# lmb-freiburg/flownet2

Hardware: AMD Instinct MI355X
Metric: image-pairs/sec FlowNetC forward at 448x320 (higher is better)
Workload: dtype f32

## Files before the change

flownet2_amd/csrc/conv_mfma.hip:

```cpp
#include "mfma_tile.hpp"

namespace fn2 {
namespace cv {

using namespace mfma;

struct Args {
  const float* in; const float* wp; const float* bias; float* out;
  int N, Cin, Hin, Win, in_ctot, in_c0;
  int Cout, Hout, Wout, out_ctot, out_c0;
  int pad;
  int nchunks;
  int ksteps;
  int tx, ty;
  int ng;
  unsigned total;
  unsigned nbig;
  float slope; int relu;
};

template <int KS_, int S_, int MW_, int NP_, int WM_, int WNX_, int WNY_, int CQ_, int P16_ = 0, int PIN_ = 0>
struct Cfg : Window<((P16_ ? 1 : 4) * WNY_ - 1) * S_ + KS_,
                    ((P16_ ? 16 : 4) * NP_ * WNX_ - 1) * S_ + KS_ + 4,
                    CQ_, WM_ * WNX_ * WNY_> {
  static constexpr int KS = KS_, S = S_, MW = MW_, NP = NP_, WM = WM_, WNX = WNX_, WNY = WNY_, CQ = CQ_, P16 = P16_;
  static constexpr int PIN = PIN_;
  static constexpr int NW = WM * WNX * WNY, THREADS = 64 * NW;
  static constexpr int PADL = 4;
  static constexpr int TW = (P16 ? 16 : 4) * NP * WNX, TH = (P16 ? 1 : 4) * WNY;
  static_assert(!P16 || (KS == 1 && S == 1), "row tiles are for 1x1 kernels");
  static_assert(Cfg::WR == (TH - 1) * S + KS && Cfg::WC == (TW - 1) * S + KS + PADL, "window of the tile");
  static constexpr int KSC = CQ * KS * KS;
  static constexpr int NBUFA = ring_depth(KSC);
  static_assert(KSC % NBUFA == 0, "ring phase must repeat per chunk");
  static_assert(2 * Cfg::BUF * 4 <= 160 * 1024, "LDS");
};

template <class K>
__device__ __forceinline__ void conv_body(const Args& a, int g, int bx, int by, int n) {
  static_assert(K::THREADS == 256, "launch bounds");
  extern __shared__ __attribute__((aligned(16))) float smem[];
  constexpr int KS = K::KS, S = K::S, MW = K::MW, NP = K::NP;
  const int tid = threadIdx.x, lane = tid & 63;
  const int wave = __builtin_amdgcn_readfirstlane(tid >> 6);
  const int wm = wave % K::WM, wnx = (wave / K::WM) % K::WNX, wny = wave / (K::WM * K::WNX);
  const int x0 = bx * K::TW, y0 = by * K::TH;

  const size_t plane = (size_t)a.Hin * a.Win;
  const __amdgpu_buffer_rsrc_t rs = nchw_rsrc(a.in, n, a.in_ctot, a.in_c0, a.Cin, plane);
  unsigned voff[K::RPW];
  window_plan<K>(voff, wave, lane, S * y0 - a.pad, S * x0 - K::PADL, a.Hin, a.Win, plane);
  const unsigned lds_base = (unsigned)(uintptr_t)(lds_ptr_t)smem;
  const unsigned chunk_bytes = 4u * 4u * K::CQ * (unsigned)plane;
  auto stage = [&](int chunk, int buf) { stage_chunk<K>(rs, voff, lds_base + 4u * (unsigned)(buf * K::BUF), wave, (unsigned)chunk * chunk_bytes); };

  const int kq = lane >> 4, p16 = lane & 15, py = K::P16 ? 0 : p16 >> 2, px = K::P16 ? p16 : p16 & 3;
  constexpr int PW = K::P16 ? 16 : 4, PH = K::P16 ? 1 : 4;
  const int bbase = kq * K::CS + (S * (PH * wny + py)) * K::RS + S * (PW * NP * wnx + px) + K::PADL - a.pad;
  using WV = typename WVec<MW>::T;
  const int cg0 = (g * K::WM + wm) * MW;
  const float* wl = weight_lane(a.wp, cg0, a.ksteps, lane);

  f32x4 acc[MW][NP];
#pragma unroll
  for (int j = 0; j < MW; ++j)
#pragma unroll
    for (int p = 0; p < NP; ++p) acc[j][p] = f32x4{0.f, 0.f, 0.f, 0.f};

  WV wreg[K::NBUFA];
  stage(0, 0);
#pragma unroll
  for (int i = 0; i < K::NBUFA - 1; ++i) wreg[i] = weight_load<MW>(wl, i);

  for (int c = 0; c < a.nchunks; ++c) {
    const int buf = c & 1;
    wait_vmcnt<K::NBUFA - 1>();
    __builtin_amdgcn_s_barrier();
    if (c + 1 < a.nchunks) stage(c + 1, buf ^ 1);
    const float* win = smem + buf * K::BUF + bbase;
    const int ks0 = c * K::KSC;
    if constexpr (K::PIN) {
      float b[2][NP];
      auto tap_off = [](int ks) { const int cq = ks / (KS * KS), ky = (ks / KS) % KS, kx = ks % KS; return cq * 4 * K::CS + ky * K::RS + kx; };
#pragma unroll
      for (int p = 0; p < NP; ++p) b[0][p] = win[tap_off(0) + PW * S * p];
      __builtin_amdgcn_sched_barrier(0);
#pragma unroll
      for (int ks = 0; ks < K::KSC; ++ks) {
        wreg[(ks + K::NBUFA - 1) % K::NBUFA] = weight_load<MW>(wl, ks0 + ks + K::NBUFA - 1);
        const WV w = wreg[ks % K::NBUFA];
#pragma unroll
        for (int p = 0; p < NP; ++p) {
#pragma unroll
          for (int j = 0; j < MW; ++j) acc[j][p] = __builtin_amdgcn_mfma_f32_16x16x4f32(b[ks & 1][p], wget<MW>(w, j), acc[j][p], 0, 0, 0);
          if (ks + 1 < K::KSC) b[(ks + 1) & 1][p] = win[tap_off(ks + 1 < K::KSC ? ks + 1 : ks) + PW * S * p];
          __builtin_amdgcn_sched_barrier(0);
        }
      }
    } else {
#pragma unroll
    for (int ks = 0; ks < K::KSC; ++ks) {
      wreg[(ks + K::NBUFA - 1) % K::NBUFA] = weight_load<MW>(wl, ks0 + ks + K::NBUFA - 1);
      const int cq = ks / (KS * KS), ky = (ks / KS) % KS, kx = ks % KS;
      float b[NP];
#pragma unroll
      for (int p = 0; p < NP; ++p) b[p] = win[cq * 4 * K::CS + ky * K::RS + kx + PW * S * p];
      const WV w = wreg[ks % K::NBUFA];
#pragma unroll
      for (int j = 0; j < MW; ++j)
#pragma unroll
        for (int p = 0; p < NP; ++p) acc[j][p] = __builtin_amdgcn_mfma_f32_16x16x4f32(b[p], wget<MW>(w, j), acc[j][p], 0, 0, 0);
    }
    }
  }

  const int y = K::P16 ? y0 + wny : y0 + 4 * wny + (lane >> 4);
  if (y < a.Hout) {
#pragma unroll
    for (int j = 0; j < MW; ++j) {
      const int co = 16 * (cg0 + j) + (lane & 15);
      const float bv = a.bias ? a.bias[co] : 0.f;
      float* orow = a.out + (((size_t)n * a.out_ctot + a.out_c0 + co) * a.Hout + y) * a.Wout;
#pragma unroll
      for (int p = 0; p < NP; ++p) {
        const int x = K::P16 ? x0 + 16 * (NP * wnx + p) + 4 * (lane >> 4) : x0 + 4 * (NP * wnx + p);
        store_row4(orow, x, a.Wout, acc[j][p], bv, a.relu, a.slope);
      }
    }
  }
}

__device__ __forceinline__ void decode_tile(const Args& a, unsigned t, int& g, int& bx, int& by, int& n) {
  g = t % a.ng; t /= a.ng;
  bx = t % a.tx; t /= a.tx;
  by = t % a.ty;
  n = t / a.ty;
}

template <class K>
__global__ void __launch_bounds__(256, 2)
conv_mfma(Args a) {
  unsigned t;
  if (!xcd_task(blockIdx.x, a.total, t)) return;
  int g, bx, by, n;
  decode_tile(a, t, g, bx, by, n);
  conv_body<K>(a, g, bx, by, n);
}

template <class K>
__global__ void __launch_bounds__(256, 2)
conv_mfma_tail(Args a) {
  using KH = Cfg<K::KS, K::S, K::MW / 2, K::NP, K::WM, K::WNX, K::WNY, K::CQ, K::P16>;
  int g, bx, by, n;
  if (blockIdx.x < a.nbig) {
    const unsigned t = (blockIdx.x % 8) * (a.nbig / 8) + blockIdx.x / 8;
    decode_tile(a, t, g, bx, by, n);
    conv_body<K>(a, g, bx, by, n);
  } else {
    unsigned u;
    if (!xcd_task(blockIdx.x - a.nbig, 2 * (a.total - a.nbig), u)) return;
    decode_tile(a, a.nbig + u / 2, g, bx, by, n);
    conv_body<KH>(a, 2 * g + (int)(u & 1), bx, by, n);
  }
}

__global__ void pack_weights(const float* __restrict__ w, float* __restrict__ wp, int Cout, int Cin, int KS, int ksteps, int kalloc) {
  const long long total = (long long)((Cout + 63) / 64) * kalloc * 256;
  for (long long i = blockIdx.x * (long long)blockDim.x + threadIdx.x; i < total; i += (long long)gridDim.x * blockDim.x) {
    const int j = (int)(i & 3), lane = (int)((i >> 2) & 63);
    long long r = i >> 8;
    const int ks = (int)(r % kalloc), grp = (int)(r / kalloc);
    const int co = 64 * grp + 16 * j + (lane & 15), kq = lane >> 4;
    const int cq = ks / (KS * KS), tap = ks % (KS * KS);
    const int ci = 4 * cq + kq;
    float v = 0.f;
    if (ks < ksteps && ci < Cin && co < Cout) v = w[((size_t)co * Cin + ci) * KS * KS + tap];
    wp[i] = v;
  }
}

template <int KS> struct PackTile {
  static constexpr int T = KS * KS;
  static constexpr int QT = KS == 1 ? 8 : KS == 3 ? 3 : KS == 4 ? 2 : 1;
  static constexpr int CIL = 4 * QT, ROW = CIL * T + 1;
  static constexpr int LDS_FLOATS = 64 * ROW;
};

template <int KS, int ORDER>
__global__ void __launch_bounds__(256) pack_weights_view(const float* __restrict__ w, float* __restrict__ wp, int ksteps, int kalloc,
                                                         int src_co, int src_ci, long long s_co, long long s_ci, int flip) {
  using P = PackTile<KS>;
  constexpr int T = P::T, QT = P::QT, CIL = P::CIL, ROW = P::ROW;
  __shared__ float tile[P::LDS_FLOATS];
  const int grp = blockIdx.x, cq0 = blockIdx.y * QT;
  const int co0 = 64 * grp, ci0 = 4 * cq0;
  const int nquads = ksteps / T;
  constexpr int TOTAL = 64 * CIL * T;
  if constexpr (ORDER == 0) {
    const float* src = w + (size_t)co0 * s_co + (size_t)ci0 * T;
#pragma unroll
    for (int i = threadIdx.x; i < TOTAL; i += 256) {
      const int col = i / (CIL * T), e = i - col * (CIL * T), c = e / T;
      tile[col * ROW + e] = (co0 + col < src_co && ci0 + c < src_ci) ? src[(size_t)col * s_co + e] : 0.f;
    }
  } else if constexpr (ORDER == 1) {
    const float* src = w + (size_t)ci0 * s_ci + (size_t)co0 * T;
#pragma unroll
    for (int i = threadIdx.x; i < TOTAL; i += 256) {
      const int c = i / (64 * T), e = i - c * (64 * T), col = e / T, t = e - col * T;
      tile[col * ROW + c * T + t] = (co0 + col < src_co && ci0 + c < src_ci) ? src[(size_t)c * s_ci + e] : 0.f;
    }
  } else {
#pragma unroll
    for (int i = threadIdx.x; i < TOTAL; i += 256) {
      const int col = i / (CIL * T), e = i - col * (CIL * T), c = e / T, t = e - c * T;
      tile[col * ROW + e] = (co0 + col < src_co && ci0 + c < src_ci) ? w[(size_t)(co0 + col) * s_co + (size_t)(ci0 + c) * s_ci + t] : 0.f;
    }
  }
  __syncthreads();
  const int nq = min(QT, nquads - cq0);
  float* dst = wp + ((size_t)grp * kalloc + (size_t)cq0 * T) * 256;
  const int j = threadIdx.x & 3, lane = threadIdx.x >> 2;
  const float* trow = tile + (16 * j + (lane & 15)) * ROW + (lane >> 4) * T;
#pragma unroll
  for (int ks = 0; ks < QT * T; ++ks) {
    const int cq = ks / T, tap = ks - cq * T;
    if (cq < nq) dst[ks * 256 + threadIdx.x] = trow[4 * cq * T + (flip ? T - 1 - tap : tap)];
  }
  if (cq0 + QT >= nquads)
    for (int i = threadIdx.x; i < (kalloc - ksteps) * 256; i += 256) wp[((size_t)grp * kalloc + ksteps) * 256 + i] = 0.f;
}

template <int KS>
static void launch_pack_view(const float* w, float* wp, int Cout, int ksteps, int kalloc, int src_co, int src_ci, long long s_co, long long s_ci, int flip,
                             hipStream_t st) {
  using P = PackTile<KS>;
  const dim3 grid((unsigned)((Cout + 63) / 64), (unsigned)cdiv(ksteps / P::T, P::QT));
  if (s_ci == (long long)P::T) hipLaunchKernelGGL((pack_weights_view<KS, 0>), grid, dim3(256), 0, st, w, wp, ksteps, kalloc, src_co, src_ci, s_co, s_ci, flip);
  else if (s_co == (long long)P::T) hipLaunchKernelGGL((pack_weights_view<KS, 1>), grid, dim3(256), 0, st, w, wp, ksteps, kalloc, src_co, src_ci, s_co, s_ci, flip);
  else hipLaunchKernelGGL((pack_weights_view<KS, 2>), grid, dim3(256), 0, st, w, wp, ksteps, kalloc, src_co, src_ci, s_co, s_ci, flip);
}

constexpr int kSpare = 8;
constexpr int kChunkQuads = 2;

inline int chunk_quads(int KS) { return KS == 1 ? 8 : kChunkQuads; }
inline int ksteps_for(int Cin, int KS) { return cdiv(cdiv(Cin, 4), chunk_quads(KS)) * chunk_quads(KS) * KS * KS; }

template <class K>
static void set_geometry(Args& a) {
  if constexpr (K::P16) {
    a.Win *= a.Hin; a.Hin = 1; a.Wout *= a.Hout; a.Hout = 1;
  }
  a.tx = cdiv(a.Wout, K::TW); a.ty = cdiv(a.Hout, K::TH);
  a.ng = a.Cout / (16 * K::MW * K::WM);
  a.nchunks = cdiv(cdiv(a.Cin, 4), K::CQ);
}

inline long long tiles_of(const Args& a) { return (long long)a.N * a.tx * a.ty * a.ng; }

template <class K>
static int launch(const Args& base, hipStream_t st) {
  Args a = base;
  set_geometry<K>(a);
  if (tiles_of(a) > 0x3fffff00ll) return fail(FN2_ERR_UNSUPPORTED, "conv_mfma: grid too large");
  a.total = (unsigned)tiles_of(a); a.nbig = a.total;
  const unsigned grid = 8 * ((a.total + 7) / 8);
  constexpr size_t lds = sizeof(float) * 2 * K::BUF;
  set_dynamic_lds_once<&conv_mfma<K>>((int)lds);
  hipLaunchKernelGGL((conv_mfma<K>), dim3(grid), dim3(K::THREADS), lds, st, a);
  return check_launch("conv_mfma_forward");
}

inline unsigned whole_rounds(long long tiles) { return (unsigned)(tiles / 256 * 256); }

template <class K>
static int launch_tail(const Args& base, hipStream_t st) {
  if constexpr (K::MW < 2) {
    return fail(FN2_ERR_UNSUPPORTED, "conv_mfma: variant has no split tail");
  } else {
    Args a = base;
    set_geometry<K>(a);
    if (tiles_of(a) > 0x1fffff00ll) return fail(FN2_ERR_UNSUPPORTED, "conv_mfma: grid too large");
    a.total = (unsigned)tiles_of(a); a.nbig = whole_rounds(a.total);
    const unsigned nsm = 2 * (a.total - a.nbig);
    const unsigned grid = a.nbig + 8 * ((nsm + 7) / 8);
    constexpr size_t lds = sizeof(float) * 2 * K::BUF;
    set_dynamic_lds_once<&conv_mfma_tail<K>>((int)lds);
    hipLaunchKernelGGL((conv_mfma_tail<K>), dim3(grid), dim3(K::THREADS), lds, st, a);
    return check_launch("conv_mfma_forward");
  }
}

struct Variant {
  int ks, s, mw, np, wm, wnx, wny, p16;
  int (*fn)(const Args&, hipStream_t);
  int (*fn_tail)(const Args&, hipStream_t);
};

#define FN2_CV_LIST(X) \
   \
  X(1, 1, 2, 7, 2, 2, 1, 8, 1) X(1, 1, 2, 7, 2, 1, 2, 8, 1) X(1, 1, 4, 7, 1, 2, 2, 8, 0) X(1, 1, 4, 7, 1, 1, 4, 8, 0) X(1, 1, 2, 6, 2, 2, 1, 8, 1) \
  X(1, 1, 2, 4, 2, 2, 1, 8, 1) X(1, 1, 2, 7, 1, 2, 2, 8, 0) X(1, 1, 2, 7, 1, 4, 1, 8, 0) X(1, 1, 2, 4, 1, 2, 2, 8, 0) X(1, 1, 4, 4, 1, 2, 2, 8, 0) \
   \
  X(3, 1, 2, 7, 2, 2, 1, 2, 1) X(3, 1, 2, 7, 2, 1, 2, 2, 1) X(3, 1, 4, 7, 1, 2, 2, 2, 0) X(3, 1, 4, 7, 1, 1, 4, 2, 0) \
  X(3, 1, 2, 6, 2, 2, 1, 2, 1) X(3, 1, 4, 6, 1, 2, 2, 2, 0) X(3, 1, 4, 4, 1, 2, 2, 2, 0) X(3, 1, 2, 4, 2, 2, 1, 2, 1) \
   \
  X(3, 2, 2, 7, 2, 1, 2, 2, 1) X(3, 2, 4, 7, 1, 1, 4, 2, 0) X(3, 2, 2, 6, 2, 2, 1, 2, 1) X(3, 2, 4, 6, 1, 2, 2, 2, 0) X(3, 2, 2, 4, 2, 2, 1, 2, 1) \
   \
  X(4, 2, 2, 7, 2, 2, 1, 2, 1) X(4, 2, 2, 7, 2, 1, 2, 2, 1) X(4, 2, 4, 7, 1, 2, 2, 2, 0) X(4, 2, 2, 6, 2, 2, 1, 2, 1) X(4, 2, 4, 4, 1, 2, 2, 2, 0) X(4, 2, 2, 4, 2, 2, 1, 2, 1) \
   \
  X(5, 2, 2, 7, 2, 2, 1, 1, 1) X(5, 2, 2, 7, 2, 1, 2, 1, 1) X(5, 2, 4, 7, 1, 2, 2, 1, 0) X(5, 2, 4, 7, 1, 1, 4, 1, 0) \
  X(5, 2, 2, 6, 2, 2, 1, 1, 1) X(5, 2, 4, 6, 1, 2, 2, 1, 0) X(5, 2, 4, 4, 1, 2, 2, 1, 0) \
   \
  X(7, 2, 2, 6, 2, 2, 1, 1, 1) X(7, 2, 2, 7, 2, 2, 1, 1, 1) X(7, 2, 4, 4, 1, 2, 2, 1, 0) X(7, 2, 4, 6, 1, 2, 2, 1, 0) X(7, 2, 2, 4, 2, 2, 1, 1, 1)

template <class K, int TAIL> struct TailFn { static constexpr int (*fn)(const Args&, hipStream_t) = nullptr; };
template <class K> struct TailFn<K, 1> { static constexpr int (*fn)(const Args&, hipStream_t) = &launch_tail<K>; };

#define FN2_CV_ROW(KS, S, MW, NP, WM, WNX, WNY, CQ, TAIL) \
  {KS, S, MW, NP, WM, WNX, WNY, 0, &launch<Cfg<KS, S, MW, NP, WM, WNX, WNY, CQ>>, TailFn<Cfg<KS, S, MW, NP, WM, WNX, WNY, CQ>, TAIL>::fn},
#define FN2_CV_ROW16(MW, NP, WM, WNX, WNY, TAIL) \
  {1, 1, MW, NP, WM, WNX, WNY, 1, &launch<Cfg<1, 1, MW, NP, WM, WNX, WNY, 8, 1>>, TailFn<Cfg<1, 1, MW, NP, WM, WNX, WNY, 8, 1>, TAIL>::fn},
#define FN2_CV_PIN(KS, S, MW, NP, WM, WNX, WNY, CQ, P16, TAIL) \
  {KS, S, MW, NP, WM, WNX, WNY, P16, &launch<Cfg<KS, S, MW, NP, WM, WNX, WNY, CQ, P16, 1>>, TailFn<Cfg<KS, S, MW, NP, WM, WNX, WNY, CQ, P16, 1>, TAIL>::fn},
static const Variant kVariants[] = {FN2_CV_LIST(FN2_CV_ROW)
  FN2_CV_ROW16(2, 7, 2, 2, 1, 1) FN2_CV_ROW16(2, 7, 4, 1, 1, 1) FN2_CV_ROW16(4, 7, 1, 4, 1, 0) FN2_CV_ROW16(4, 7, 2, 2, 1, 0) FN2_CV_ROW16(2, 5, 2, 2, 1, 1)
  FN2_CV_ROW16(2, 4, 2, 2, 1, 1) FN2_CV_ROW16(2, 7, 1, 4, 1, 0) FN2_CV_ROW16(2, 5, 1, 4, 1, 0) FN2_CV_ROW16(4, 5, 1, 4, 1, 0) FN2_CV_ROW16(2, 4, 1, 4, 1, 0)
  FN2_CV_ROW16(4, 5, 2, 2, 1, 0) FN2_CV_ROW16(4, 4, 2, 2, 1, 0)
  FN2_CV_ROW16(2, 9, 4, 1, 1, 1) FN2_CV_ROW16(2, 9, 2, 2, 1, 1) FN2_CV_ROW16(2, 3, 2, 2, 1, 1) FN2_CV_ROW16(4, 3, 1, 4, 1, 0)
  FN2_CV_ROW16(4, 9, 4, 1, 1, 0) FN2_CV_ROW16(4, 9, 2, 2, 1, 0) FN2_CV_ROW16(4, 7, 4, 1, 1, 0)
  FN2_CV_PIN(5, 2, 2, 7, 2, 2, 1, 1, 0, 1) FN2_CV_PIN(5, 2, 2, 7, 2, 1, 2, 1, 0, 1)
  FN2_CV_PIN(1, 1, 4, 9, 4, 1, 1, 8, 1, 0) FN2_CV_PIN(1, 1, 2, 9, 4, 1, 1, 8, 1, 1) FN2_CV_PIN(1, 1, 2, 5, 2, 2, 1, 8, 1, 1) FN2_CV_PIN(1, 1, 4, 7, 4, 1, 1, 8, 1, 0)
  FN2_CV_PIN(1, 1, 2, 7, 2, 2, 1, 8, 1, 1) FN2_CV_PIN(1, 1, 2, 3, 2, 2, 1, 8, 1, 1)
  FN2_CV_PIN(3, 1, 2, 7, 2, 2, 1, 2, 0, 1) FN2_CV_PIN(3, 1, 2, 6, 2, 2, 1, 2, 0, 1) FN2_CV_PIN(3, 2, 2, 7, 2, 1, 2, 2, 0, 1) FN2_CV_PIN(3, 2, 2, 6, 2, 2, 1, 2, 0, 1)
  FN2_CV_PIN(4, 2, 2, 7, 2, 2, 1, 2, 0, 1) FN2_CV_PIN(4, 2, 2, 6, 2, 2, 1, 2, 0, 1) FN2_CV_PIN(5, 2, 2, 6, 2, 2, 1, 1, 0, 1)
  FN2_CV_PIN(7, 2, 2, 6, 2, 2, 1, 1, 0, 1) FN2_CV_PIN(7, 2, 4, 6, 1, 2, 2, 1, 0, 0)};
constexpr int kNumVariants = sizeof(kVariants) / sizeof(kVariants[0]);

int g_forced_variant = -1;

static double variant_cost(const Variant& v, const Args& a, bool tail) {
  const int tw = (v.p16 ? 16 : 4) * v.np * v.wnx, th = (v.p16 ? 1 : 4) * v.wny;
  const long long wgs = v.p16 ? (long long)a.N * cdiv(a.Wout * a.Hout, tw) * (a.Cout / (16 * v.mw * v.wm))
                              : (long long)a.N * cdiv(a.Wout, tw) * cdiv(a.Hout, th) * (a.Cout / (16 * v.mw * v.wm));
  double rounds = (double)((wgs + 255) / 256);
  if (tail) {
    const long long r = wgs % 256;
    if (wgs < 256 || r == 0 || r > 128) return 1e30;
    rounds = (double)(wgs / 256) + 0.5 * 1.12;
  }
  const double eff = 1.0 / (1.0 + 0.08 * (4.0 / v.mw - 1.0) + 0.02 * (7.0 / v.np - 1.0));
  return rounds * v.mw * v.np / eff;
}

static bool variant_applies(const Variant& v, const Args& a, int KS, int S) {
  if (!v.p16 && a.Win % 4 != 0) return false;
  return v.ks == KS && v.s == S && a.Cout % (16 * v.mw * v.wm) == 0;
}

}
}

using namespace fn2;

FN2_API size_t fn2_conv_mfma_packed_floats(int Cout, int Cin, int kernel) {
  if (Cout <= 0 || Cout % 32 != 0 || Cin <= 0 || kernel <= 0) return 0;
  return (size_t)((Cout + 63) / 64) * (cv::ksteps_for(Cin, kernel) + cv::kSpare) * 256;
}

FN2_API int fn2_conv_mfma_pack_weights_view(const float* weight, float* packed, int Cout, int Cin, int kernel, int src_cout, int src_cin,
                                            long long stride_cout, long long stride_cin, int flip, void* stream);

FN2_API int fn2_conv_mfma_pack_weights(const float* weight, float* packed, int Cout, int Cin, int kernel, void* stream) {
  if (!weight || !packed) return fail(FN2_ERR_INVALID_ARG, "conv_mfma_pack_weights: null blob");
  if (Cout <= 0 || Cout % 32 != 0 || Cin <= 0 || (kernel != 1 && kernel != 3 && kernel != 4 && kernel != 5 && kernel != 7))
    return fail(FN2_ERR_UNSUPPORTED, "conv_mfma_pack_weights: needs Cout %% 32 == 0 and kernel_size 1, 3, 4, 5 or 7 (got Cout %d, kernel %d)", Cout, kernel);
  return fn2_conv_mfma_pack_weights_view(weight, packed, Cout, Cin, kernel, Cout, Cin, (long long)Cin * kernel * kernel, (long long)kernel * kernel, 0, stream);
}

FN2_API int fn2_conv_mfma_pack_weights_view(const float* weight, float* packed, int Cout, int Cin, int kernel, int src_cout, int src_cin,
                                            long long stride_cout, long long stride_cin, int flip, void* stream) {
  if (!weight || !packed) return fail(FN2_ERR_INVALID_ARG, "conv_mfma_pack_weights_view: null blob");
  if (Cout <= 0 || Cout % 32 != 0 || Cin <= 0 || (kernel != 1 && kernel != 3 && kernel != 4 && kernel != 5 && kernel != 7))
    return fail(FN2_ERR_UNSUPPORTED, "conv_mfma_pack_weights_view: needs Cout %% 32 == 0 and kernel_size 1, 3, 4, 5 or 7 (got Cout %d, kernel %d)", Cout, kernel);
  if (src_cout < 1 || src_cout > Cout || src_cin < 1 || src_cin > Cin || stride_cout < 1 || stride_cin < 1)
    return fail(FN2_ERR_INVALID_ARG, "conv_mfma_pack_weights_view: bad source view (%d of %d, %d of %d channels, strides %lld / %lld)", src_cout, Cout,
                src_cin, Cin, stride_cout, stride_cin);
  const int ksteps = cv::ksteps_for(Cin, kernel), kalloc = ksteps + cv::kSpare;
  hipStream_t st = as_stream(stream);
  switch (kernel) {
    case 1: cv::launch_pack_view<1>(weight, packed, Cout, ksteps, kalloc, src_cout, src_cin, stride_cout, stride_cin, flip ? 1 : 0, st); break;
    case 3: cv::launch_pack_view<3>(weight, packed, Cout, ksteps, kalloc, src_cout, src_cin, stride_cout, stride_cin, flip ? 1 : 0, st); break;
    case 4: cv::launch_pack_view<4>(weight, packed, Cout, ksteps, kalloc, src_cout, src_cin, stride_cout, stride_cin, flip ? 1 : 0, st); break;
    case 5: cv::launch_pack_view<5>(weight, packed, Cout, ksteps, kalloc, src_cout, src_cin, stride_cout, stride_cin, flip ? 1 : 0, st); break;
    default: cv::launch_pack_view<7>(weight, packed, Cout, ksteps, kalloc, src_cout, src_cin, stride_cout, stride_cin, flip ? 1 : 0, st); break;
  }
  return check_launch("conv_mfma_pack_weights_view");
}

FN2_API int fn2_conv_mfma_supported(int Cin, int Hin, int Win, int Cout, int kernel, int stride, int pad) {
  if (Cin <= 0 || Hin <= 0 || Win <= 0 || Cout <= 0 || Cout % 32 != 0) return 0;
  if (kernel == 1 ? ((long long)Hin * Win) % 4 != 0 : Win % 4 != 0) return 0;
  if (!((kernel == 1 && stride == 1) || (kernel == 3 && (stride == 1 || stride == 2)) || (kernel == 4 && stride == 2) || (kernel == 5 && stride == 2) || (kernel == 7 && stride == 2))) return 0;
  if (pad < 0 || pad > 4 || pad > kernel - 1) return 0;
  if ((long long)Cin * Hin * Win >= (1ll << 28)) return 0;
  const int Hout = (Hin + 2 * pad - kernel) / stride + 1, Wout = (Win + 2 * pad - kernel) / stride + 1;
  if (Hout < 1 || Wout < 1) return 0;
  cv::Args a{};
  a.Win = Win; a.Cout = Cout;
  for (int i = 0; i < cv::kNumVariants; ++i)
    if (cv::variant_applies(cv::kVariants[i], a, kernel, stride)) return 1;
  return 0;
}

FN2_API int fn2_debug_set_conv_variant(int v) { cv::g_forced_variant = v; return FN2_OK; }
FN2_API int fn2_conv_mfma_num_variants(void) { return cv::kNumVariants; }

FN2_API int fn2_conv_mfma_forward(const float* bottom, const float* packed_weight, const float* bias, float* top,
                                  int N, int Cin, int Hin, int Win, int bottom_channels, int bottom_c0,
                                  int Cout, int top_channels, int top_c0, int kernel, int stride, int pad,
                                  int relu, float negative_slope, void* stream) {
  if (N < 0) return fail(FN2_ERR_INVALID_ARG, "conv_mfma: bad batch");
  if (N == 0) return FN2_OK;
  if (const int rc = mfma::check_conv_args("conv_mfma", bottom, packed_weight, top, Cin, bottom_channels, bottom_c0, Cout, top_channels, top_c0, [&] {
        return fn2_conv_mfma_supported(Cin, Hin, Win, Cout, kernel, stride, pad) ? FN2_OK
            : fail(FN2_ERR_UNSUPPORTED, "conv_mfma: unsupported geometry (Cin %d, %dx%d, Cout %d, k %d s %d p %d)", Cin, Hin, Win, Cout, kernel, stride, pad);
      }))
    return rc;
  cv::Args a{};
  a.in = bottom; a.wp = packed_weight; a.bias = bias; a.out = top;
  a.N = N; a.Cin = Cin; a.Hin = Hin; a.Win = Win; a.in_ctot = bottom_channels; a.in_c0 = bottom_c0;
  a.Cout = Cout; a.Hout = (Hin + 2 * pad - kernel) / stride + 1; a.Wout = (Win + 2 * pad - kernel) / stride + 1;
  a.out_ctot = top_channels; a.out_c0 = top_c0; a.pad = pad;
  a.ksteps = cv::ksteps_for(Cin, kernel) + cv::kSpare;
  a.slope = negative_slope; a.relu = relu;
  hipStream_t st = as_stream(stream);
  static TuneCache cache("conv_mfma", cv::kNumVariants);
  const TuneKey key{N, Cin, Hin, Win, Cout, kernel, stride, pad, bottom_channels == Cin, top_channels == Cout};
  mfma::Pick p;
  if (const int rc = mfma::pick_variant(p, "conv_mfma", cv::g_forced_variant, cv::kNumVariants, true, cache, key, st,
                                        [&](int i) { return cv::variant_applies(cv::kVariants[i], a, kernel, stride); },
                                        [&](int i, bool tail) { return cv::variant_cost(cv::kVariants[i], a, tail); },
                                        [&](int i, bool tail) { return tail ? cv::kVariants[i].fn_tail(a, st) : cv::kVariants[i].fn(a, st); },
                                        [&](int i) { return cv::kVariants[i].fn_tail != nullptr; }))
    return rc;
  return p.tail ? cv::kVariants[p.variant].fn_tail(a, st) : cv::kVariants[p.variant].fn(a, st);
}
```

flownet2_amd/csrc/mfma_tile.hpp:

```cpp
#pragma once

#include "autotune.hpp"
#include "fn2_common.hpp"

namespace fn2 {
namespace mfma {

using f32x4 = __attribute__((ext_vector_type(4))) float;
using f32x2 = __attribute__((ext_vector_type(2))) float;
using lds_ptr_t = __attribute__((address_space(3))) void*;

constexpr int cdiv(int a, int b) { return (a + b - 1) / b; }
constexpr int up_mod(int v, int r, int m) { return v + ((r - v % m) + m) % m; }

constexpr unsigned kOOB = 0x7ffffff0u;
constexpr int kRsrcWord3 = 0x00020000;

template <int N>
__device__ __forceinline__ void wait_vmcnt() {
  asm volatile("s_waitcnt vmcnt(%0)" ::"n"(N) : "memory");
}

__device__ __forceinline__ __amdgpu_buffer_rsrc_t nchw_rsrc(const float* blob, int n, int ctot, int c0, int C, size_t plane) {
  return __builtin_amdgcn_make_buffer_rsrc(const_cast<float*>(blob + ((size_t)n * ctot + c0) * plane), 0, (unsigned)(4u * C * plane), kRsrcWord3);
}

template <int MW> struct WVec;
template <> struct WVec<1> { using T = float; };
template <> struct WVec<2> { using T = f32x2; };
template <> struct WVec<4> { using T = f32x4; };

template <int MW>
__device__ __forceinline__ float wget(const typename WVec<MW>::T& v, int j) {
  if constexpr (MW == 1) return v; else return v[j];
}

template <int WR_, int WC_, int CQ_, int NW_>
struct Window {
  static constexpr int WR = WR_, WC = WC_;
  static constexpr int RS = up_mod(cdiv(WC, 4) * 4, 4, 16);
  static constexpr int CS = up_mod(WR * RS, 16, 32);
  static constexpr int SLOTS_C = CS / 4;
  static constexpr int SLOTS = 4 * CQ_ * SLOTS_C;
  static constexpr int NRUN = cdiv(SLOTS, 64);
  static constexpr int RPW = cdiv(NRUN, NW_);
  static constexpr int BUF = NRUN * 256;
};

constexpr int ring_depth(int KSC) { return (KSC % 6 == 0) ? 6 : (KSC % 5 == 0) ? 5 : (KSC % 7 == 0) ? 7 : (KSC % 4 == 0) ? 4 : 3; }

template <class K>
__device__ __forceinline__ void window_plan(unsigned (&voff)[K::RPW], int wave, int lane, int y_first, int x_first, int Hin, int Win, size_t plane) {
#pragma unroll
  for (int i = 0; i < K::RPW; ++i) {
    const int s = (i * K::NW + wave) * 64 + lane;
    voff[i] = kOOB;
    if (s < K::SLOTS) {
      const int c = s / K::SLOTS_C, rem = s % K::SLOTS_C;
      const int row = rem / (K::RS / 4), gq = rem % (K::RS / 4);
      const int yi = y_first + row, xi = x_first + 4 * gq;
      if (row < K::WR && 4 * gq < K::WC && yi >= 0 && yi < Hin && xi >= 0 && xi < Win)
        voff[i] = 4u * (unsigned)(c * plane + (size_t)yi * Win + xi);
    }
  }
}

template <class K>
__device__ __forceinline__ void stage_chunk(__amdgpu_buffer_rsrc_t rs, const unsigned (&voff)[K::RPW], unsigned dst, int wave, unsigned soff) {
#pragma unroll
  for (int i = 0; i < K::RPW; ++i) {
    const int r = i * K::NW + wave;
    if (r < K::NRUN)
      __builtin_amdgcn_raw_ptr_buffer_load_lds(rs, (lds_ptr_t)(uintptr_t)(dst + 1024u * (unsigned)r), 16, voff[i], soff, 0, 0);
  }
}

__device__ __forceinline__ const float* weight_lane(const float* wp, int cg0, int ksteps, int lane) {
  return wp + ((size_t)(cg0 / 4) * ksteps * 64 + lane) * 4 + (cg0 % 4);
}

template <int MW>
__device__ __forceinline__ typename WVec<MW>::T weight_load(const float* wl, int ks) {
  return *reinterpret_cast<const typename WVec<MW>::T*>(wl + (size_t)ks * 256);
}

__device__ __forceinline__ bool xcd_task(unsigned block, unsigned total, unsigned& task) {
  const unsigned per_xcd = (total + 7) / 8;
  task = (block % 8) * per_xcd + block / 8;
  return !(block / 8 >= per_xcd || task >= total);
}

__device__ __forceinline__ f32x4 bias_relu4(f32x4 v, float bias, int relu, float slope) {
#pragma unroll
  for (int r = 0; r < 4; ++r) {
    float s = v[r] + bias;
    if (relu) s = s > 0.f ? s : s * slope;
    v[r] = s;
  }
  return v;
}

__device__ __forceinline__ void store4(float* orow, int x, int Wout, f32x4 v) {
  if (x + 3 < Wout) *reinterpret_cast<f32x4*>(orow + x) = v;
  else {
#pragma unroll
    for (int r = 0; r < 4; ++r) if (x + r < Wout) orow[x + r] = v[r];
  }
}

__device__ __forceinline__ void store_row4(float* orow, int x, int Wout, f32x4 v, float bias, int relu, float slope) {
  store4(orow, x, Wout, bias_relu4(v, bias, relu, slope));
}

template <auto Kernel>
inline void set_dynamic_lds_once(int bytes) {
  static bool attr_set = false;
  if (!attr_set) {
    (void)hipFuncSetAttribute(reinterpret_cast<const void*>(Kernel), hipFuncAttributeMaxDynamicSharedMemorySize, bytes);
    attr_set = true;
  }
}

template <class Geometry>
int check_conv_args(const char* what, const float* bottom, const float* packed, const float* top, int Cin, int bottom_channels, int bottom_c0,
                    int Cout, int top_channels, int top_c0, Geometry geometry) {
  if (!bottom || !packed || !top) return fail(FN2_ERR_INVALID_ARG, "%s: null blob", what);
  if (const int rc = geometry()) return rc;
  if (bottom_c0 < 0 || bottom_c0 + Cin > bottom_channels || top_c0 < 0 || top_c0 + Cout > top_channels)
    return fail(FN2_ERR_INVALID_ARG, "%s: channel slice outside the blob", what);
  if (((reinterpret_cast<uintptr_t>(bottom) | reinterpret_cast<uintptr_t>(top) | reinterpret_cast<uintptr_t>(packed)) & 15) != 0)
    return fail(FN2_ERR_UNSUPPORTED, "%s: blobs must be 16-byte aligned", what);
  return FN2_OK;
}

struct Pick { int variant = -1; bool tail = false; };

template <class Applies, class Cost, class Run, class HasTail>
int pick_variant(Pick& p, const char* what, int forced, int nvariants, bool split_tail, TuneCache& cache, const TuneKey& key, hipStream_t st,
                 Applies applies, Cost cost, Run run, HasTail has_tail) {
  p = Pick{};
  if (forced >= 0) {
    p.tail = split_tail && forced >= 1000;
    p.variant = split_tail ? forced % 1000 : forced;
    if (p.variant >= nvariants || !applies(p.variant) || (p.tail && !has_tail(p.variant)))
      return fail(FN2_ERR_UNSUPPORTED, "%s: forced variant %d does not apply", what, forced);
    return FN2_OK;
  }
  int picked = -1;
  if (autotune_enabled(st)) {
    auto usable = [&](int c) -> bool {
      const int i = split_tail ? c / 2 : c;
      return applies(i) && (!(split_tail && (c & 1)) || (has_tail(i) && cost(i, true) < 1e29));
    };
    picked = autotune_pick(cache, key, split_tail ? 2 * nvariants : nvariants, st, [&](int c) -> int {
      return usable(c) ? run(split_tail ? c / 2 : c, split_tail && (c & 1)) : FN2_ERR_UNSUPPORTED;
    }, usable);
  }
  if (picked >= 0) {
    p.variant = split_tail ? picked / 2 : picked;
    p.tail = split_tail && (picked & 1);
  } else {
    double bc = 0;
    for (int i = 0; i < nvariants; ++i) {
      if (!applies(i)) continue;
      for (int t = 0; t < (split_tail && has_tail(i) ? 2 : 1); ++t) {
        const double c = cost(i, t == 1);
        if (p.variant < 0 || c < bc) { p.variant = i; bc = c; p.tail = t == 1; }
      }
    }
  }
  if (p.variant < 0) return fail(FN2_ERR_UNSUPPORTED, "%s: no kernel variant for this geometry", what);
  return FN2_OK;
}

}
}
```

Before: 3524.

## Manage weight prefetch ring with explicit vmcnt waits via inline asm loads

Replaces compiler-generated weight loads with inline-asm global loads using an SGPR base and per-lane VGPR offset. Each ring slot now gets an explicit s_waitcnt sized to the number of loads still in flight, counting the LDS staging DMA, so the compiler no longer inserts conservative vmcnt(0) waits. The last chunk skips prefetches beyond the end, with branches chosen at run time. The intent is to keep weight prefetches in flight during the MFMA loop. The risk is that inline asm hides dependencies from the compiler, so a miscounted wait would read stale registers.

```diff
diff --git a/flownet2_amd/csrc/conv_mfma.hip b/flownet2_amd/csrc/conv_mfma.hip
--- a/flownet2_amd/csrc/conv_mfma.hip
+++ b/flownet2_amd/csrc/conv_mfma.hip
@@ -59,7 +59,8 @@
   const int bbase = kq * K::CS + (S * (PH * wny + py)) * K::RS + S * (PW * NP * wnx + px) + K::PADL - a.pad;
   using WV = typename WVec<MW>::T;
   const int cg0 = (g * K::WM + wm) * MW;
-  const float* wl = weight_lane(a.wp, cg0, a.ksteps, lane);
+  const float* wb = a.wp + (size_t)(cg0 / 4) * a.ksteps * 256 + (cg0 % 4);
+  const unsigned wlane = 16u * (unsigned)lane;
 
   f32x4 acc[MW][NP];
 #pragma unroll
@@ -67,16 +68,32 @@
 #pragma unroll
     for (int p = 0; p < NP; ++p) acc[j][p] = f32x4{0.f, 0.f, 0.f, 0.f};
 
+  constexpr int R = K::NBUFA - 1, DMA = K::NRUN / K::NW;
+  static_assert(R + DMA <= 63, "vmcnt has 6 bits");
   WV wreg[K::NBUFA];
   stage(0, 0);
-#pragma unroll
-  for (int i = 0; i < K::NBUFA - 1; ++i) wreg[i] = weight_load<MW>(wl, i);
+  if (a.nchunks > 0) {
+#pragma unroll
+    for (int i = 0; i < R; ++i) wreg[i] = weight_fetch<MW>(wb + (size_t)i * 256, wlane);
+  }
+  auto weight_step = [&](int ks0, int ks, int rest) -> WV {
+    const float* wks = wb + (size_t)(ks0 + ks + R) * 256;
+    if (ks + R < K::KSC) wreg[(ks + R) % K::NBUFA] = weight_fetch<MW>(wks, wlane);
+    else wreg[(ks + R) % K::NBUFA] = weight_fetch_unless_last<MW>(rest, wks, wlane);
+    const int left = K::KSC - 1 - ks < R ? K::KSC - 1 - ks : R;
+    if (ks < R) ring_wait_either(rest, left, R + DMA);
+    else if (left < R) ring_wait_either(rest, left, R);
+    else ring_wait(R);
+    weight_landed(wreg[ks % K::NBUFA]);
+    return wreg[ks % K::NBUFA];
+  };
 
   for (int c = 0; c < a.nchunks; ++c) {
     const int buf = c & 1;
-    wait_vmcnt<K::NBUFA - 1>();
+    const int rest = a.nchunks - 1 - c;
+    wait_vmcnt<R>();
     __builtin_amdgcn_s_barrier();
-    if (c + 1 < a.nchunks) stage(c + 1, buf ^ 1);
+    if (rest) stage(c + 1, buf ^ 1);
     const float* win = smem + buf * K::BUF + bbase;
     const int ks0 = c * K::KSC;
     if constexpr (K::PIN) {
@@ -87,8 +104,7 @@
       __builtin_amdgcn_sched_barrier(0);
 #pragma unroll
       for (int ks = 0; ks < K::KSC; ++ks) {
-        wreg[(ks + K::NBUFA - 1) % K::NBUFA] = weight_load<MW>(wl, ks0 + ks + K::NBUFA - 1);
-        const WV w = wreg[ks % K::NBUFA];
+        const WV w = weight_step(ks0, ks, rest);
 #pragma unroll
         for (int p = 0; p < NP; ++p) {
 #pragma unroll
@@ -100,12 +116,11 @@
     } else {
 #pragma unroll
     for (int ks = 0; ks < K::KSC; ++ks) {
-      wreg[(ks + K::NBUFA - 1) % K::NBUFA] = weight_load<MW>(wl, ks0 + ks + K::NBUFA - 1);
+      const WV w = weight_step(ks0, ks, rest);
       const int cq = ks / (KS * KS), ky = (ks / KS) % KS, kx = ks % KS;
       float b[NP];
 #pragma unroll
       for (int p = 0; p < NP; ++p) b[p] = win[cq * 4 * K::CS + ky * K::RS + kx + PW * S * p];
-      const WV w = wreg[ks % K::NBUFA];
 #pragma unroll
       for (int j = 0; j < MW; ++j)
 #pragma unroll
@@ -114,6 +129,7 @@
     }
   }
 
+  wait_vmcnt<0>();
   const int y = K::P16 ? y0 + wny : y0 + 4 * wny + (lane >> 4);
   if (y < a.Hout) {
 #pragma unroll
diff --git a/flownet2_amd/csrc/mfma_tile.hpp b/flownet2_amd/csrc/mfma_tile.hpp
--- a/flownet2_amd/csrc/mfma_tile.hpp
+++ b/flownet2_amd/csrc/mfma_tile.hpp
@@ -82,6 +82,48 @@
 template <int MW>
 __device__ __forceinline__ typename WVec<MW>::T weight_load(const float* wl, int ks) {
   return *reinterpret_cast<const typename WVec<MW>::T*>(wl + (size_t)ks * 256);
+}
+
+template <int MW>
+__device__ __forceinline__ typename WVec<MW>::T weight_fetch(const float* base, unsigned lane_bytes) {
+  typename WVec<MW>::T w;
+  if constexpr (MW == 1) asm volatile("global_load_dword %0, %1, %2" : "=v"(w) : "v"(lane_bytes), "s"(base));
+  else if constexpr (MW == 2) asm volatile("global_load_dwordx2 %0, %1, %2" : "=v"(w) : "v"(lane_bytes), "s"(base));
+  else asm volatile("global_load_dwordx4 %0, %1, %2" : "=v"(w) : "v"(lane_bytes), "s"(base));
+  return w;
+}
+
+template <class T>
+__device__ __forceinline__ void weight_landed(T& w) { asm volatile("" : "+v"(w)); }
+
+constexpr int vmcnt_clamp(int n) { return n < 63 ? n : 63; }
+
+__device__ __forceinline__ void ring_wait(int n) { asm volatile("s_waitcnt vmcnt(%0)" ::"i"(vmcnt_clamp(n))); }
+
+__device__ __forceinline__ void ring_wait_either(int rest, int n_last, int n_else) {
+  asm volatile(
+      "s_cmp_eq_u32 %0, 0\n\t"
+      "s_cbranch_scc1 .Lrwt_%=\n\t"
+      "s_waitcnt vmcnt(%2)\n\t"
+      "s_branch .Lrwe_%=\n"
+      ".Lrwt_%=:\n\t"
+      "s_waitcnt vmcnt(%1)\n"
+      ".Lrwe_%=:"
+      :
+      : "s"(rest), "i"(vmcnt_clamp(n_last)), "i"(vmcnt_clamp(n_else))
+      : "scc");
+}
+
+template <int MW>
+__device__ __forceinline__ typename WVec<MW>::T weight_fetch_unless_last(int rest, const float* base, unsigned lane_bytes) {
+  typename WVec<MW>::T w;
+#define FN2_FETCH_UNLESS(INSN) \
+  asm volatile("s_cmp_eq_u32 %3, 0\n\ts_cbranch_scc1 .Lwfs_%=\n\t" INSN " %0, %1, %2\n.Lwfs_%=:" : "=v"(w) : "v"(lane_bytes), "s"(base), "s"(rest) : "scc")
+  if constexpr (MW == 1) FN2_FETCH_UNLESS("global_load_dword");
+  else if constexpr (MW == 2) FN2_FETCH_UNLESS("global_load_dwordx2");
+  else FN2_FETCH_UNLESS("global_load_dwordx4");
+#undef FN2_FETCH_UNLESS
+  return w;
 }
 
 __device__ __forceinline__ bool xcd_task(unsigned block, unsigned total, unsigned& task) {
```

After: 3580 (median of 6 runs). 1.02x the previous value.
